# cure-lab/MagicDrive

Hardware: AMD Instinct MI355X
Metric: 6-view scenes/sec at 224x400, 50-step DDIM (higher is better)
Workload: dtype bf16; 1 GPU; configs[1]: 6-view 224x400, text-only conditioning (camera_param=None -> CFG off), 50-step DDIM, bf16; scenes_per_gpu=64, ddim_steps=50, scheduler=ddim, parallelism=scene-sharded x1, hipgraph=True, streams=2, output_type=latent

## Files before the change

### include/mdx.h

```cpp
#ifndef MDX_H_
#define MDX_H_

#include <stdint.h>

#ifdef __cplusplus
extern "C" {
#endif

#define MDX_OK 0
#define MDX_EINVAL (-1)
#define MDX_ELAUNCH (-2)
#define MDX_EUNSUPPORTED (-3)

#define MDX_ABI_VERSION 12

#define MDX_EPI_NONE 0
#define MDX_EPI_GEGLU 1
#define MDX_EPI_SILU 2

typedef struct MdxGemmDesc {
    const void* A; const void* W; void* C; const void* R;
    const float* bias; const float* temb; const int32_t* sel_ptr; float* ws;
    int64_t M, N, K;
    int64_t lda, ldw, ldc, ldr;
// ... 32 lines not shown
    const void* X; const void* Wt; void* Y; const void* R;
    const float* bias; const float* temb; const int32_t* sel_ptr; void* reserved_p;
    int64_t B, Hi, Wi, Cin, Ho, Wo, Cout;
    int64_t kh, kw, sh, sw, ph, pw;
    int64_t ldx, ldy, ldr;
    int64_t temb_sel_stride, temb_b_stride;
    int64_t epilogue, x_is_f32, y_is_f32, reserved0;
} MdxConvDirectDesc;
int mdx_conv2d_direct(const MdxConvDirectDesc* d, void* stream);

typedef struct MdxAttnDesc {
    const void* Q; const void* K; const void* Vt; void* O;
    const int32_t* kvmap; const int32_t* tk_dev;
    int64_t B, H, Tq, Tk, d, nsrc;
    int64_t ldq, sQ, ldk, sK, ldv, sV, ldo, sO;
    double scale;
    int64_t joint;
    int64_t q_prescaled;
    int64_t causal;
    int64_t v_rowmajor;
} MdxAttnDesc;
int mdx_attention_bf16(const MdxAttnDesc* d, void* stream);
int mdx_attention_ctx_rows_bf16(const MdxAttnDesc* d, void* stream);

typedef struct MdxGroupNormDesc {
    const void* X; void* Y; const float* gamma; const float* beta;
    int64_t B, HW, C, G, ldx, ldy;
    double eps;
    int64_t silu;
    float* ws; int64_t ws_bytes;
} MdxGroupNormDesc;
int mdx_groupnorm_bf16(const MdxGroupNormDesc* d, void* stream);

int mdx_groupnorm_resident_bf16(const MdxGroupNormDesc* d, void* stream);

typedef struct MdxLayerNormDesc {
    const void* X; void* Y; const float* gamma; const float* beta;
    int64_t M, C, ldx, ldy;
    double eps;
    int64_t reserved0;
} MdxLayerNormDesc;
int mdx_layernorm_bf16(const MdxLayerNormDesc* d, void* stream);

typedef struct MdxSoftmaxDesc {
    const float* X; void* Y;
    int64_t rows, T, ldx, ldy;
// ... 85 lines not shown
    int64_t n, group_elems, jump, n_rows, coef_ld, col_t, col_p, cfg, xin_c, xin_ld;
} MdxRenoiseDesc;
int mdx_latent_renoise_bf16(const MdxRenoiseDesc* d, void* stream);

#define MDX_OP_GEMM 1
#define MDX_OP_CONV 2
#define MDX_OP_CONV_DIRECT 3
#define MDX_OP_ATTN 4
#define MDX_OP_GROUPNORM 5
#define MDX_OP_LAYERNORM 6
#define MDX_OP_EW 7
#define MDX_OP_FOURIER 8
#define MDX_OP_GATHER 9
#define MDX_OP_TIMEEMB 10
#define MDX_OP_DDIM 11
#define MDX_OP_UNIPC 12
#define MDX_OP_SOFTMAX 13
#define MDX_OP_ATTN_ROWS 14
#define MDX_OP_GROUPNORM_RESIDENT 15
#define MDX_OP_GROUP_STATS 16
#define MDX_OP_SDPA 17
#define MDX_OP_LATENT_BLEND 18
#define MDX_OP_LATENT_RENOISE 19

#define MDX_DTYPE_BF16 0
#define MDX_DTYPE_F16 1

#define MDX_OP_BYTES 512
typedef struct MdxOp {
    int64_t opcode;
    int64_t dtype;
    unsigned char desc[MDX_OP_BYTES - 16];
} MdxOp;

int mdx_gemm_f16(const MdxGemmDesc* d, void* stream);
int mdx_conv2d_f16(const MdxConvDesc* d, void* stream);
int mdx_conv2d_direct_f16(const MdxConvDirectDesc* d, void* stream);
int mdx_attention_f16(const MdxAttnDesc* d, void* stream);
int mdx_groupnorm_f16(const MdxGroupNormDesc* d, void* stream);
int mdx_groupnorm_resident_f16(const MdxGroupNormDesc* d, void* stream);
int mdx_layernorm_f16(const MdxLayerNormDesc* d, void* stream);
int mdx_elementwise_f16(const MdxEwDesc* d, void* stream);
int mdx_fourier_embed_f16(const MdxFourierDesc* d, void* stream);
int mdx_gather_rows_f16(const MdxGatherDesc* d, void* stream);
int mdx_timestep_embedding_f16(const MdxTimeEmbDesc* d, void* stream);
int mdx_cfg_ddim_step_f16(const MdxDdimDesc* d, void* stream);
int mdx_cfg_unipc_step_f16(const MdxUniPCDesc* d, void* stream);
int mdx_softmax_rows_f16(const MdxSoftmaxDesc* d, void* stream);
int mdx_attention_ctx_rows_f16(const MdxAttnDesc* d, void* stream);
int mdx_group_stats_f16(const MdxStatsDesc* d, void* stream);
int mdx_sdpa_f16(const MdxSdpaDesc* d, void* stream);
int mdx_latent_blend_f16(const MdxBlendDesc* d, void* stream);
int mdx_latent_renoise_f16(const MdxRenoiseDesc* d, void* stream);

int mdx_program_run(const MdxOp* ops, int64_t n, void* stream);

int mdx_graph_create(const MdxOp* ops, int64_t n, void** graph_out);
int mdx_graph_launch(void* graph, void* stream);
int mdx_graph_destroy(void* graph);

int mdx_abi_version(void);
const char* mdx_build_id(void);
const char* mdx_last_error(void);
const char* mdx_last_kernel(void);
int mdx_set_option(const char* key, int64_t value);
int mdx_get_option(const char* key, int64_t* value_out);
const char* mdx_option_name(int64_t index);

int mdx_device_info(int64_t* out3);

#ifdef __cplusplus
}
#endif
#endif
```

### magicdrive_amd/_lib.py

```python
from __future__ import annotations

import ctypes as C
import os
from typing import Dict, List, Tuple

_HERE = os.path.dirname(os.path.abspath(__file__))
LIB_PATH = os.environ.get("MDX_LIB_PATH") or os.path.join(_HERE, "libmdx.so")

ABI_VERSION = 12

OP_GEMM, OP_CONV, OP_CONV_DIRECT, OP_ATTN, OP_GROUPNORM, OP_LAYERNORM = 1, 2, 3, 4, 5, 6
OP_EW, OP_FOURIER, OP_GATHER, OP_TIMEEMB, OP_DDIM, OP_UNIPC, OP_SOFTMAX = 7, 8, 9, 10, 11, 12, 13
OP_ATTN_ROWS = 14
OP_GROUPNORM_RESIDENT = 15
OP_GROUP_STATS = 16
OP_SDPA = 17
OP_LATENT_BLEND = 18
OP_LATENT_RENOISE = 19
OP_BYTES = 512

EPI_NONE, EPI_GEGLU, EPI_SILU = 0, 1, 2
EW_ADD, EW_COPY, EW_UPSAMPLE, EW_NCHW_TO_NHWC, EW_NHWC_TO_NCHW, EW_SILU, EW_SCALE = 1, 2, 3, 4, 5, 6, 7

P, I, D = C.c_void_p, C.c_int64, C.c_double


def _struct(name: str, fields: List[Tuple[str, object]]):
    return type(name, (C.Structure,), {"_fields_": fields})


def _f(kind, names: str):
    return [(n, kind) for n in names.split()]


MdxGemmDesc = _struct("MdxGemmDesc", _f(P, "A W C R bias temb sel_ptr ws") + _f(I, "M N K lda ldw ldc ldr batch sA sW sC sR "
                      "temb_sel_stride temb_b_stride rows_per_b epilogue splitk c_is_f32 ws_bytes") + _f(P, "Vt") + _f(I, "vt_from vt_T vt_ld vt_stride")
                      + _f(D, "ln_eps") + _f(P, "ln_csum ln_scratch") + _f(P, "rowstat_out") + _f(I, "rowstat_parts") + _f(P, "ln_stats") + _f(I, "ln_stats_parts") + _f(P, "Wq"))
MdxConvDesc = _struct("MdxConvDesc", _f(P, "X Wt Y R bias temb sel_ptr ws") + _f(I, "B Hi Wi Cin Ho Wo Cout kh kw sh sw ph pw "
                      "ldx ldy ldr temb_sel_stride temb_b_stride epilogue splitk ws_bytes upsample2x"))
MdxConvDirectDesc = _struct("MdxConvDirectDesc", _f(P, "X Wt Y R bias temb sel_ptr reserved_p") + _f(I, "B Hi Wi Cin Ho Wo Cout kh kw sh sw ph pw "
                            "ldx ldy ldr temb_sel_stride temb_b_stride epilogue x_is_f32 y_is_f32 reserved0"))
# ... 12 lines not shown

MdxSoftmaxDesc = _struct("MdxSoftmaxDesc", _f(P, "X Y") + _f(I, "rows T ldx ldy") + _f(D, "scale") + _f(I, "reserved0"))
MdxStatsDesc = _struct("MdxStatsDesc", _f(P, "X out row_dev") + _f(I, "G n sG n_rows f32"))
MdxSdpaDesc = _struct("MdxSdpaDesc", _f(P, "Q K V O klen_dev") + _f(I, "B H Tq Tk d ldq sQ ldk sK ldv sV ldo sO") + _f(D, "scale") + _f(I, "causal"))
MdxBlendDesc = _struct("MdxBlendDesc", _f(P, "x cond noise mask coef step_ptr x_in") + _f(I, "n mask_elems coef_ld col_a col_s last_step cfg xin_c xin_ld"))
MdxRenoiseDesc = _struct("MdxRenoiseDesc", _f(P, "x x_in coef step_ptr visit_ptr seeds") + _f(I, "n group_elems jump n_rows coef_ld col_t col_p cfg xin_c xin_ld"))
DESC_OF_OP = {
    OP_GEMM: MdxGemmDesc, OP_CONV: MdxConvDesc, OP_CONV_DIRECT: MdxConvDirectDesc, OP_ATTN: MdxAttnDesc,
    OP_GROUPNORM: MdxGroupNormDesc, OP_LAYERNORM: MdxLayerNormDesc, OP_EW: MdxEwDesc, OP_FOURIER: MdxFourierDesc,
    OP_GATHER: MdxGatherDesc, OP_TIMEEMB: MdxTimeEmbDesc, OP_DDIM: MdxDdimDesc, OP_UNIPC: MdxUniPCDesc, OP_SOFTMAX: MdxSoftmaxDesc,
}
DTYPE_BF16, DTYPE_F16 = 0, 1
ENTRY_OF_OP = {
    OP_GEMM: "mdx_gemm_bf16", OP_CONV: "mdx_conv2d_bf16", OP_CONV_DIRECT: "mdx_conv2d_direct", OP_ATTN: "mdx_attention_bf16",
    OP_GROUPNORM: "mdx_groupnorm_bf16", OP_LAYERNORM: "mdx_layernorm_bf16", OP_EW: "mdx_elementwise",
    OP_FOURIER: "mdx_fourier_embed", OP_GATHER: "mdx_gather_rows", OP_TIMEEMB: "mdx_timestep_embedding", OP_DDIM: "mdx_cfg_ddim_step",
    OP_UNIPC: "mdx_cfg_unipc_step", OP_SOFTMAX: "mdx_softmax_rows",
    OP_ATTN_ROWS: "mdx_attention_ctx_rows_bf16",
    OP_GROUPNORM_RESIDENT: "mdx_groupnorm_resident_bf16",
    OP_GROUP_STATS: "mdx_group_stats_bf16",
    OP_SDPA: "mdx_sdpa_bf16",
    OP_LATENT_BLEND: "mdx_latent_blend_bf16",
    OP_LATENT_RENOISE: "mdx_latent_renoise_bf16",
}
def entry_name(opcode: int, dtype: int = DTYPE_BF16) -> str:
    n = ENTRY_OF_OP[opcode]
    if dtype == DTYPE_BF16:
        return n
    return (n[:-5] if n.endswith("_bf16") else n) + "_f16"


EXPORTS = sorted(set(ENTRY_OF_OP.values()) | {entry_name(o, DTYPE_F16) for o in ENTRY_OF_OP} | {
    "mdx_program_run", "mdx_graph_create", "mdx_graph_launch", "mdx_graph_destroy",
    "mdx_abi_version", "mdx_build_id", "mdx_last_error", "mdx_last_kernel", "mdx_device_info", "mdx_set_option", "mdx_get_option", "mdx_option_name"})


class MdxOp(C.Structure):
    _fields_ = [("opcode", I), ("dtype", I), ("desc", C.c_ubyte * (OP_BYTES - 16))]


assert C.sizeof(MdxOp) == OP_BYTES
for _d in list(DESC_OF_OP.values()) + [MdxStatsDesc, MdxSdpaDesc, MdxBlendDesc, MdxRenoiseDesc]:
    assert C.sizeof(_d) <= OP_BYTES - 16 and C.sizeof(_d) % 8 == 0


class MdxError(RuntimeError):
# ... 142 lines not shown
```

### magicdrive_amd/csrc/api.hip

```cpp
#include <cstring>
#include <mutex>
#include <set>
#include <utility>
#include "launch.h"
#include "options.h"
#include <atomic>
#include <cstdlib>

namespace mdx_rt {
char* error_buffer() {
    static thread_local char buf[512] = {0};
    return buf;
}
char* kernel_tag_buffer() {
    static thread_local char buf[128] = {0};
    return buf;
}
int ensure_dyn_smem(const void* kernel, size_t bytes, const char* what) {
    static std::mutex mu;
    static std::set<std::pair<const void*, int>> done;
    int dev = 0;
    hipError_t e = hipGetDevice(&dev);
    if (e != hipSuccess) return mdx::set_error(MDX_ELAUNCH, "hipGetDevice: %s", hipGetErrorString(e));
    std::lock_guard<std::mutex> lk(mu);
// ... 58 lines not shown
static int run_op(const MdxOp* op, hipStream_t st) {
    const void* d = op->desc;
    if (op->dtype == MDX_DTYPE_F16) {
        switch (op->opcode) {
            case MDX_OP_GEMM: return mdx_gemm_f16((const MdxGemmDesc*)d, st);
            case MDX_OP_CONV: return mdx_conv2d_f16((const MdxConvDesc*)d, st);
            case MDX_OP_CONV_DIRECT: return mdx_conv2d_direct_f16((const MdxConvDirectDesc*)d, st);
            case MDX_OP_ATTN: return mdx_attention_f16((const MdxAttnDesc*)d, st);
            case MDX_OP_GROUPNORM: return mdx_groupnorm_f16((const MdxGroupNormDesc*)d, st);
            case MDX_OP_GROUPNORM_RESIDENT: return mdx_groupnorm_resident_f16((const MdxGroupNormDesc*)d, st);
            case MDX_OP_LAYERNORM: return mdx_layernorm_f16((const MdxLayerNormDesc*)d, st);
            case MDX_OP_EW: return mdx_elementwise_f16((const MdxEwDesc*)d, st);
            case MDX_OP_FOURIER: return mdx_fourier_embed_f16((const MdxFourierDesc*)d, st);
            case MDX_OP_GATHER: return mdx_gather_rows_f16((const MdxGatherDesc*)d, st);
            case MDX_OP_TIMEEMB: return mdx_timestep_embedding_f16((const MdxTimeEmbDesc*)d, st);
            case MDX_OP_DDIM: return mdx_cfg_ddim_step_f16((const MdxDdimDesc*)d, st);
            case MDX_OP_UNIPC: return mdx_cfg_unipc_step_f16((const MdxUniPCDesc*)d, st);
            case MDX_OP_SOFTMAX: return mdx_softmax_rows_f16((const MdxSoftmaxDesc*)d, st);
            case MDX_OP_ATTN_ROWS: return mdx_attention_ctx_rows_f16((const MdxAttnDesc*)d, st);
            case MDX_OP_GROUP_STATS: return mdx_group_stats_f16((const MdxStatsDesc*)d, st);
            case MDX_OP_SDPA: return mdx_sdpa_f16((const MdxSdpaDesc*)d, st);
            case MDX_OP_LATENT_BLEND: return mdx_latent_blend_f16((const MdxBlendDesc*)d, st);
            case MDX_OP_LATENT_RENOISE: return mdx_latent_renoise_f16((const MdxRenoiseDesc*)d, st);
            default: return set_error(MDX_EINVAL, "unknown opcode %ld", (long)op->opcode);
        }
    }
    if (op->dtype != MDX_DTYPE_BF16) return set_error(MDX_EINVAL, "MdxOp.dtype %ld: 0 (bf16) or 1 (fp16)", (long)op->dtype);
    switch (op->opcode) {
        case MDX_OP_GEMM: return mdx_gemm_bf16((const MdxGemmDesc*)d, st);
        case MDX_OP_CONV: return mdx_conv2d_bf16((const MdxConvDesc*)d, st);
        case MDX_OP_CONV_DIRECT: return mdx_conv2d_direct((const MdxConvDirectDesc*)d, st);
        case MDX_OP_ATTN: return mdx_attention_bf16((const MdxAttnDesc*)d, st);
        case MDX_OP_GROUPNORM: return mdx_groupnorm_bf16((const MdxGroupNormDesc*)d, st);
        case MDX_OP_GROUPNORM_RESIDENT: return mdx_groupnorm_resident_bf16((const MdxGroupNormDesc*)d, st);
        case MDX_OP_LAYERNORM: return mdx_layernorm_bf16((const MdxLayerNormDesc*)d, st);
        case MDX_OP_EW: return mdx_elementwise((const MdxEwDesc*)d, st);
        case MDX_OP_FOURIER: return mdx_fourier_embed((const MdxFourierDesc*)d, st);
        case MDX_OP_GATHER: return mdx_gather_rows((const MdxGatherDesc*)d, st);
        case MDX_OP_TIMEEMB: return mdx_timestep_embedding((const MdxTimeEmbDesc*)d, st);
        case MDX_OP_DDIM: return mdx_cfg_ddim_step((const MdxDdimDesc*)d, st);
        case MDX_OP_UNIPC: return mdx_cfg_unipc_step((const MdxUniPCDesc*)d, st);
        case MDX_OP_SOFTMAX: return mdx_softmax_rows((const MdxSoftmaxDesc*)d, st);
        case MDX_OP_ATTN_ROWS: return mdx_attention_ctx_rows_bf16((const MdxAttnDesc*)d, st);
        case MDX_OP_GROUP_STATS: return mdx_group_stats_bf16((const MdxStatsDesc*)d, st);
        case MDX_OP_SDPA: return mdx_sdpa_bf16((const MdxSdpaDesc*)d, st);
        case MDX_OP_LATENT_BLEND: return mdx_latent_blend_bf16((const MdxBlendDesc*)d, st);
        case MDX_OP_LATENT_RENOISE: return mdx_latent_renoise_bf16((const MdxRenoiseDesc*)d, st);
        default: return set_error(MDX_EINVAL, "unknown opcode %ld", (long)op->opcode);
    }
}

extern "C" int mdx_program_run(const MdxOp* ops, int64_t n, void* stream) {
    if (!ops && n > 0) return set_error(MDX_EINVAL, "mdx_program_run: null program");
    for (int64_t i = 0; i < n; ++i) {
        int rc = run_op(&ops[i], (hipStream_t)stream);
        if (rc != MDX_OK) {
            char tmp[400];
            strncpy(tmp, error_buffer(), sizeof(tmp) - 1);
            tmp[sizeof(tmp) - 1] = 0;
            return set_error(rc, "op %ld (opcode %ld): %s", (long)i, (long)ops[i].opcode, tmp);
        }
    }
    return MDX_OK;
}

struct GraphHandle {
    hipGraph_t graph;
    hipGraphExec_t exec;
};

// ... 61 lines not shown
```

### magicdrive_amd/csrc/options.h

```cpp
#pragma once
#include <cstdint>

namespace mdx_rt {
int64_t opt(int id);
}

namespace mdx {

#define MDX_OPTIONS(X) \
    X(ATTN_SWZ, 2, "XCD-aware block order of attention.hip: 0 off, 1 per (view, head), 2 per view (all heads of a view on one XCD)") \
    X(ATTN_NW4_BLOCKS, 256L, "attention.hip: 4-wave workgroups from this many blocks") \
    X(ATTN_NW8_BLOCKS, (1L << 40), "attention.hip: 8-wave workgroups from this many blocks") \
    X(ATTN_NW, 0, "force the waves per workgroup of attention.hip (0 = heuristic)") \
    X(ATTN2, 1, "attention2.hip for head dim 40") \
    X(ATTN3, 0, "only in `make ATTN3=1` builds: tools/attn3/attention3.hip (permute-free P, QK of the next kv tile beside this tile's softmax) for the head-dim-40 FOLD launches: self, cross-view, joint") \
    X(ATTN3_WGS, 0, "attention3.hip: persistent workgroups per XCD (0 = automatic: two per CU)") \
    X(ATTN2_PF, 1, "attention2.hip, head dim 40 FOLD 32-query form: permute-free P (PV on 32x32x16 MFMAs, K rows permuted so that a lane's scores are its PV operand)") \
    X(ATTN2_D80, 2, "attention2.hip for head dim 80: 0 never, 1 always, 2 only the two-source cross-view form") \
    X(ATTN2_FOLD, 1, "attention2.hip: subtract the running maximum inside the QK MFMA when Q is pre-scaled (head dim 40)") \
    X(ATTN2_RES, 1, "attention2.hip: kv sequences of <= 3 tiles (text context) resident in LDS, one workgroup per (view, head) walks the query blocks: 0 off, 1 for launches of >= 1024 (view, head) pairs, 2 whenever supported") \
    X(ATTN2_VIEWMAP, 1, "attention2.hip block order: 1 = all heads and query blocks of a view on one XCD (a row's 128-byte lines are shared by the heads), 0 = per (view, head)") \
    X(ATTN2_QT, 0, "32-query tiles per wave in attention2.hip: 0 = automatic (2; 1 for one-source FOLD launches), 1 / 2 = force") \
    X(CONV_OUT_WS, 1, "direct conv with Cout <= 4 and a long K (conv_out): weight-stationary K-parallel kernel (weights in registers, 16 pixels per wave)") \
    X(GEMM_SWZ, 1, "XCD-aware tile order of the generic kernel") \
// ... 10 lines not shown
    X(XL_GEGLU320, 0, "K = 320 GEGLU on the 256-wide XL tile instead of gemm_ws.hip") \
    X(GEMM_BM256, 0, "generic 256x128 8-wave tile from M >= value (0 = never)") \
    X(GEMM_TIMING, 0, "s_memtime stamps of the generic kernel into the op workspace") \
    X(GEMM_BK, 64, "generic tile slab depth (64 or 32)") \
    X(GEMM_FLATTEN, 1, "batched shared-A GEMM as ONE col_split XL launch") \
    X(CONV_CIMAJOR, 1, "channel-block-major K order of implicit-GEMM convs") \
    X(WS_SLOTS, 512, "workgroup slots the gemm_ws M walkers are sized for") \
    X(XL_TIMING, 0, "per-workgroup s_memtime stamps into the op workspace") \
    X(GN_REVERSE, 1, "two-stage GroupNorm: statistics pass reads the tensor back to front (Infinity-Cache reuse between producer / passes)") \
    X(GN_FINALIZE_CHUNKS, 16, "two-stage GroupNorm: with more chunks per image than this the chunk partials are combined once by gn_finalize_kernel (0 = always in the apply pass)") \
    X(GN_ONE_KERNEL_ELEMS, (4L << 20), "GroupNorm tensors of at most this many elements (all images) take the one-launch kernel (one workgroup per (image, group)) instead of the two streaming passes") \
    X(GN_TWO_STAGE, 1, "streaming two-stage GroupNorm for maps >= 32768 elements") \
    X(GN_RESIDENT, 1, "register-resident one-read GroupNorm (gn_resident_kernel, an op of its own: MDX_OP_GROUPNORM_RESIDENT): 0 off (the engine emits none, the entry point refuses), 1 where gn_route.h says so (tensors above GN_ONE_KERNEL_ELEMS), 2 whenever the kernel can serve the shape") \
    X(GN_RESIDENT_K, 0, "force the groups per workgroup of gn_resident_kernel (0 = gn_route.h: the widest block that fits; tools/gn_bench.py sweeps it)") \
    X(XL_PERSIST, 1, "256x256 XL GEMMs (plain / GEGLU, optional residual) on the persistent kernel gemm_xlp_kernel") \
    X(XD, 0, "W-direct persistent GEMM (gemm_xd.hip: weights global -> registers, finished tile stored under the next tile's main loop) for the 256x256 XL GEMMs whose descriptor carries Wq (K % 128 == 0, K >= 640); bit-identical to gemm_xlp_kernel, measured 0.89-1.04x of it (profiles/r06_xd_ab.log): off by default") \
    X(XL_RASTER, 2, "XL tile order: 0 row-major, 1 XCD-strided M-tiles, 2 XCD-blocked (M-group x N-group panels per XCD)") \
    X(XL_GM, 0, "XL_RASTER 2: force the M-tiles per panel (0 = cost model, xl_layout.h: raster_shape)") \
    X(XL_GN, 0, "XL_RASTER 2: force the N-tiles per panel (0 = cost model)") \
    X(STREAMS, 2, "host side (pipeline): HIP streams a pipe() call spreads its scene chunks over (chunks of >= 16 scenes, one plan + hipGraph each)") \
    X(PLAN_CACHE, 6, "host side (pipeline): sampler plans (captured graphs + buffers) kept per pipeline (LRU); a multi-stream call pins one plan per chunk") \
    X(CHECK_TIMESTEPS, 0, "host side (schedulers): 1 = a device-resident timestep that is not in the scheduler's list raises (one sync per step) instead of poisoning the sample with NaN") \
    X(LN_FUSE, 1, "MdxGemmDesc.ln_eps: 1 = gemm_ws.hip normalises the rows in-kernel, 0 = always normalise into ln_scratch first (A/B)") \
    X(LN_STATS, 1, "MdxGemmDesc.rowstat_out / ln_stats: 1 = row statistics travel from the producer's store phase to the fused LayerNorm, 0 = round-5 behaviour (nothing emitted, in-kernel sums, GEGLU through ln_scratch) (A/B)")

enum Opt : int {
#define MDX_OPT_ENUM(key, dflt, doc) OPT_##key,
    MDX_OPTIONS(MDX_OPT_ENUM)
#undef MDX_OPT_ENUM
    OPT_COUNT
};

using mdx_rt::opt;

}
```

### magicdrive_amd/engine.py

```python
from __future__ import annotations

from typing import Dict, List, Optional, Sequence, Tuple

import torch

from . import _lib as L
from . import gn_route as GR
from . import ops as O
from . import packing as PK
from .networks.spec import heads_at

BF16, F32 = torch.bfloat16, torch.float32


def q_prescale(head_dim: int) -> float:
    return float(head_dim) ** -0.5 * 1.4426950408889634


class PackedNet:

    def __init__(self, sd: Dict[str, torch.Tensor], device, dtype=BF16):
        assert dtype in (torch.bfloat16, torch.float16), "the kernels take bf16 or fp16 operands (fp32 accumulate)"
        self.sd = sd
        self.device = device
        self.dtype = dtype
        self.cache: Dict[Tuple, torch.Tensor] = {}

    def has(self, key: str) -> bool:
        return key in self.sd

# ... 192 lines not shown
    def bhwc(self):
        return self.parent.bhwc[..., self.c0:self.c0 + self.C]

    @property
    def btc(self):
        return self.parent.btc[..., self.c0:self.c0 + self.C]


def upsample_conv_folds(device, fold, Hi: int, Wi: int, Ho: int, Wo: int, cin: int, B: int = 0, ldx: int = 0) -> bool:
    if fold is None:
        fold = torch.device(device).type == "cuda"
    if not (bool(fold) and cin % 64 == 0 and Hi * Wi + 256 < (1 << 24) and PK.upsample_fold_ok(Hi, Ho) and PK.upsample_fold_ok(Wi, Wo)):
        return False
    if B and (Ho != 2 * Hi or Wo != 2 * Wi) and (B * Hi * Wi + Wi + 2) * (ldx or cin) * 2 >= 0x7fff0000:
        return False
    return True


class Builder:

    fold_upsample = None

    gn_resident = None

    def __init__(self, cfg, device, n_views: int, n_cam: int, ws_mb: int = 64, dtype=BF16):
        self.cfg = cfg
        self.device = device
        self.B = n_views
        self.n_cam = n_cam
        self.dtype = dtype
        self.pool = Pool(device, dtype)
        self.ops: List[object] = []
        self.ctx_tk_dev: Optional[torch.Tensor] = None
        self.ctx_tk_per_view = False
        self.ws = torch.empty(ws_mb * 1024 * 1024 // 4, dtype=F32, device=device)
        self.groups = cfg["norm_num_groups"]
        self.eps = cfg["norm_eps"]
        pair = cfg["neighboring_view_pair"]
        pair = {int(k): [int(x) for x in v] for k, v in pair.items()}
        self.nattn = cfg.get("neighboring_attn_type", "add")
        if self.nattn not in ("add", "concat", "self"):
            raise NotImplementedError(f"Unknown type: {self.nattn}")
        counts = [len(pair[c]) for c in range(n_cam)]
        self.xv_counts: Optional[List[int]] = None
        self.xv_bo_scale = 1.0
        if self.nattn == "add":
# ... 144 lines not shown
        M = B * T
        if fuse_ln:
            n1 = self.pool.get(tuple(h.shape))
            ao = self.self_like_attention(net, pre + "attn1.", h, B, T, C, heads, False, name + ".attn1", ln_pre=pre + "norm1.", ln_scratch=n1, ln_stats=h_stats)
            self.pool.put(h_stats)
        else:
            n1 = self.layernorm(net, pre + "norm1.", h, name + ".norm1")
            ao = self.self_like_attention(net, pre + "attn1.", n1, B, T, C, heads, False, name + ".attn1")
        self.pool.put(n1)
        s1 = self.rowstat(M) if fuse_ln else None
        h1 = self.gemm(ao, net.lin(pre + "attn1.to_out.0.weight"), C, bias=net.vec(pre + "attn1.to_out.0.bias"), R=h, rowstat=s1, name=name + ".attn1.out")
        self.pool.put(ao); self.pool.put(h)
        if fuse_ln:
            n2 = self.pool.get(tuple(h1.shape))
            w, b, cs = net.ln_lin([pre + "attn2.to_q.weight"], pre + "norm2.", (q_prescale(C // heads),))
            q2 = self.gemm(h1, w, C, bias=b, ln_eps=1e-5, ln_csum=cs, ln_scratch=n2, ln_stats=s1, name=name + ".attn2.ln+q")
            self.pool.put(s1)
        else:
            n2 = self.layernorm(net, pre + "norm2.", h1, name + ".norm2")
            q2 = self.gemm(n2, net.lin(pre + "attn2.to_q.weight", q_prescale(C // heads)), C, name=name + ".attn2.q")
        self.pool.put(n2)
        Kc, Vtc, S = ctx_kv[pre + "attn2."]
        ao2 = self.pool.get((B * T, C))
        self.emit(O.Attn(q2.view(B, T, C), Kc, Vtc, ao2.view(B, T, C), heads=heads, Tk=S, scale=(C // heads) ** -0.5, q_prescaled=True,
                         tk_dev=None if self.ctx_tk_per_view else self.ctx_tk_dev, tk_rows=self.ctx_tk_dev if self.ctx_tk_per_view else None,
                         name=name + ".attn2"))
        self.pool.put(q2)
        has4 = net.has(pre + "attn4.to_q.weight")
        fold3 = fuse_ln and self.FOLD_NORM3 and not (has4 and self.xv_counts is not None)
        s2 = self.rowstat(M) if (fuse_ln and (has4 or fold3)) else None
        h2 = self.gemm(ao2, net.lin(pre + "attn2.to_out.0.weight"), C, bias=net.vec(pre + "attn2.to_out.0.bias"), R=h1, rowstat=s2, name=name + ".attn2.out")
        self.pool.put(ao2); self.pool.put(h1)
        s3 = s2
        if has4:
            if fuse_ln:
                n4 = self.pool.get(tuple(h2.shape))
                ao4 = self.self_like_attention(net, pre + "attn4.", h2, B, T, C, heads, True, name + ".attn4", ln_pre=pre + "norm4.", ln_scratch=n4, ln_stats=s2)
                self.pool.put(s2)
            else:
                n4 = self.layernorm(net, pre + "norm4.", h2, name + ".norm4")
                ao4 = self.self_like_attention(net, pre + "attn4.", n4, B, T, C, heads, True, name + ".attn4")
            self.pool.put(n4)
            bo_scale = self.xv_bo_scale
            zero_linear = net.has(pre + "connector.weight")
            alpha_key = pre + "connector.alpha" if net.has(pre + "connector.alpha") else None
            if self.xv_counts is not None:
                if zero_linear:
                    wf, tab = net.folded_affine_rows(pre + "connector.weight", pre + "connector.bias", pre + "attn4.to_out.0.weight", pre + "attn4.to_out.0.bias", self.xv_counts)
                else:
# ... 208 lines not shown
```

### magicdrive_amd/ops.py

```python
from __future__ import annotations

from dataclasses import dataclass, field
from typing import Optional

import torch

from . import _lib as L

BF16 = torch.bfloat16
F16 = torch.float16
H16 = (BF16, F16)
F32 = torch.float32


def _p(t: Optional[torch.Tensor]):
    return None if t is None else t.data_ptr()


def _chk(cond: bool, msg: str):
    if not cond:
        raise ValueError(msg)


def _rows2d(t: torch.Tensor):
# ... 234 lines not shown
            if self.ws is not None:
                d.ws = _p(self.ws); d.ws_bytes = self.ws.numel() * self.ws.element_size()
        return self.opcode, d


@dataclass
class Attn:
    Q: torch.Tensor
    K: torch.Tensor
    Vt: torch.Tensor
    O: torch.Tensor
    heads: int
    Tk: int
    scale: float
    kvmap: Optional[torch.Tensor] = None
    nsrc: int = 1
    name: str = ""
    joint: bool = False
    q_prescaled: bool = False
    causal: bool = False
    v_rowmajor: bool = False
    tk_dev: Optional[torch.Tensor] = None
    tk_rows: Optional[torch.Tensor] = None
    opcode = L.OP_ATTN

    def lower(self):
        Q, K, Vt, O = self.Q, self.K, self.Vt, self.O
        B, Tq, Cc = Q.shape
        _chk(Q.stride(2) == 1 and K.stride(2) == 1 and O.stride(2) == 1 and Vt.stride(2) == 1, f"attn {self.name}: inner strides")
        if self.v_rowmajor:
            _chk(Cc % self.heads == 0 and K.shape[2] == Cc and Vt.shape[2] == Cc and O.shape == Q.shape, f"attn {self.name}: shapes")
            _chk(K.shape[1] == self.Tk and Vt.shape[1] == self.Tk and Vt.shape[0] == K.shape[0], f"attn {self.name}: kv shapes")
        else:
            _chk(not self.causal, f"attn {self.name}: causal needs v_rowmajor")
            _chk(Cc % self.heads == 0 and K.shape[2] == Cc and Vt.shape[1] == Cc and O.shape == Q.shape, f"attn {self.name}: shapes")
            _chk(K.shape[1] == self.Tk and Vt.shape[2] >= self.Tk and Vt.shape[0] == K.shape[0], f"attn {self.name}: kv shapes")
        d = L.MdxAttnDesc()
        d.Q, d.K, d.Vt, d.O = _p(Q), _p(K), _p(Vt), _p(O)
        if self.kvmap is not None:
            _chk(self.kvmap.dtype == torch.int32 and self.kvmap.numel() == B * self.nsrc, f"attn {self.name}: kvmap")
            d.kvmap = _p(self.kvmap)
        else:
            _chk(self.nsrc == 1 and K.shape[0] == B, f"attn {self.name}: identity kv map needs Bkv == B")
        d.B, d.H, d.Tq, d.Tk, d.d, d.nsrc = B, self.heads, Tq, self.Tk, Cc // self.heads, self.nsrc
        d.ldq, d.sQ = Q.stride(1), Q.stride(0)
        d.ldk, d.sK = K.stride(1), K.stride(0)
        d.ldv, d.sV = Vt.stride(1), Vt.stride(0)
        d.ldo, d.sO = O.stride(1), O.stride(0)
        d.scale = float(self.scale)
        d.joint = int(self.joint)
        d.q_prescaled = int(self.q_prescaled)
        d.causal, d.v_rowmajor = int(self.causal), int(self.v_rowmajor)
        if self.tk_dev is not None:
            _chk(self.tk_dev.dtype == torch.int32 and self.tk_dev.numel() == 1 and self.tk_dev.device == Q.device,
                 f"attn {self.name}: tk_dev must be one int32 on the device of Q")
            _chk(self.nsrc == 1 and self.kvmap is None and not self.joint and not self.causal and not self.v_rowmajor,
                 f"attn {self.name}: tk_dev serves one source, no joint softmax, no causal mask, the V^T operand")
            d.tk_dev = _p(self.tk_dev)
        opcode = self.opcode
        if self.tk_rows is not None:
            _chk(self.tk_dev is None, f"attn {self.name}: tk_rows and tk_dev are mutually exclusive")
            _chk(self.tk_rows.dtype == torch.int32 and self.tk_rows.dim() == 1 and self.tk_rows.numel() == B and self.tk_rows.is_contiguous()
                 and self.tk_rows.device == Q.device, f"attn {self.name}: tk_rows must be int32 [B={B}], contiguous, on the device of Q")
            _chk(self.nsrc == 1 and self.kvmap is None and not self.joint and not self.causal and not self.v_rowmajor,
                 f"attn {self.name}: tk_rows serves one source, no joint softmax, no causal mask, the V^T operand")
            d.tk_dev = _p(self.tk_rows)
            opcode = L.OP_ATTN_ROWS
        _chk(self.nsrc >= 1 and (self.nsrc <= 8 if self.joint else self.nsrc <= 2), f"attn {self.name}: nsrc={self.nsrc} (joint={self.joint})")
        return opcode, d


@dataclass
class GroupNorm:
    X: torch.Tensor
    Y: torch.Tensor
    gamma: torch.Tensor
    beta: torch.Tensor
    groups: int
    eps: float
    silu: bool = False
    ws: Optional[torch.Tensor] = None
    name: str = ""
    opcode = L.OP_GROUPNORM

    def lower(self):
        B, HW, Cc = self.X.shape
        _chk(self.X.stride(2) == 1 and self.Y.stride(2) == 1 and self.Y.shape == self.X.shape, f"gn {self.name}: layout")
        _chk(B == 1 or (self.X.stride(0) == HW * self.X.stride(1) and self.Y.stride(0) == HW * self.Y.stride(1)), f"gn {self.name}: batch stride")
        _chk(self.gamma.dtype == F32 and self.beta.dtype == F32 and self.gamma.numel() == Cc, f"gn {self.name}: affine")
        d = L.MdxGroupNormDesc()
        d.X, d.Y, d.gamma, d.beta = _p(self.X), _p(self.Y), _p(self.gamma), _p(self.beta)
# ... 447 lines not shown
```

Measured before the change: 7.774 scenes/s.

## Add dedicated whole-row text cross-attention kernel for short key lengths

```diff
diff --git a/include/mdx.h b/include/mdx.h
--- a/include/mdx.h
+++ b/include/mdx.h
@@ -78,6 +78,7 @@
 } MdxAttnDesc;
 int mdx_attention_bf16(const MdxAttnDesc* d, void* stream);
 int mdx_attention_ctx_rows_bf16(const MdxAttnDesc* d, void* stream);
+int mdx_attention_text_bf16(const MdxAttnDesc* d, void* stream);
 
 typedef struct MdxGroupNormDesc {
     const void* X; void* Y; const float* gamma; const float* beta;
@@ -209,6 +210,7 @@
 #define MDX_OP_SDPA 17
 #define MDX_OP_LATENT_BLEND 18
 #define MDX_OP_LATENT_RENOISE 19
+#define MDX_OP_ATTN_TEXT 20
 
 #define MDX_DTYPE_BF16 0
 #define MDX_DTYPE_F16 1
@@ -239,6 +241,7 @@
 int mdx_sdpa_f16(const MdxSdpaDesc* d, void* stream);
 int mdx_latent_blend_f16(const MdxBlendDesc* d, void* stream);
 int mdx_latent_renoise_f16(const MdxRenoiseDesc* d, void* stream);
+int mdx_attention_text_f16(const MdxAttnDesc* d, void* stream);
 
 int mdx_program_run(const MdxOp* ops, int64_t n, void* stream);
 
diff --git a/magicdrive_amd/_lib.py b/magicdrive_amd/_lib.py
--- a/magicdrive_amd/_lib.py
+++ b/magicdrive_amd/_lib.py
@@ -17,6 +17,7 @@
 OP_SDPA = 17
 OP_LATENT_BLEND = 18
 OP_LATENT_RENOISE = 19
+OP_ATTN_TEXT = 20
 OP_BYTES = 512
 
 EPI_NONE, EPI_GEGLU, EPI_SILU = 0, 1, 2
@@ -75,6 +76,7 @@
     OP_SDPA: "mdx_sdpa_bf16",
     OP_LATENT_BLEND: "mdx_latent_blend_bf16",
     OP_LATENT_RENOISE: "mdx_latent_renoise_bf16",
+    OP_ATTN_TEXT: "mdx_attention_text_bf16",
 }
 def entry_name(opcode: int, dtype: int = DTYPE_BF16) -> str:
     n = ENTRY_OF_OP[opcode]
diff --git a/magicdrive_amd/attn_text_route.py b/magicdrive_amd/attn_text_route.py
--- /dev/null
+++ b/magicdrive_amd/attn_text_route.py
@@ -0,0 +1,36 @@
+from __future__ import annotations
+
+ATT_GROUP_CH = 320
+ATT_MAX_TK = 96
+ATT_MIN_TQ = 256
+ATT_MIN_BH = 1024
+
+
+def attn_text_supported(B: int, H: int, Tq: int, Tk: int, d: int, nsrc: int, has_kvmap: bool, joint: bool, causal: bool, v_rowmajor: bool,
+                        has_tk_dev: bool, q_prescaled: bool, ldq: int, sQ: int, ldk: int, sK: int, ldv: int, sV: int, ldo: int, sO: int,
+                        alignment: int, mode: int = 1) -> bool:
+    if mode <= 0:
+        return False
+    if nsrc != 1 or has_kvmap or joint or causal:
+        return False
+    if v_rowmajor or has_tk_dev or not q_prescaled:
+        return False
+    if not (H == 8 and d in (40, 80)):
+        return False
+    if B < 1 or Tq < 1 or Tk < 1 or Tk > ATT_MAX_TK:
+        return False
+    C = H * d
+    if ldq < C or ldo < C or ldk < C or ldv < Tk:
+        return False
+    if any(v % 8 for v in (ldq, sQ, ldo, sO, ldk, sK, ldv, sV)):
+        return False
+    if alignment < 16:
+        return False
+    tiles = (Tq + 31) // 32
+    if B > 0x7fffffff // (tiles * 2):
+        return False
+    if Tq * max(ldq, ldo) >= (1 << 30):
+        return False
+    if mode >= 2:
+        return True
+    return Tq >= ATT_MIN_TQ and B * H >= ATT_MIN_BH
diff --git a/magicdrive_amd/csrc/api.hip b/magicdrive_amd/csrc/api.hip
--- a/magicdrive_amd/csrc/api.hip
+++ b/magicdrive_amd/csrc/api.hip
@@ -104,6 +104,7 @@
             case MDX_OP_SDPA: return mdx_sdpa_f16((const MdxSdpaDesc*)d, st);
             case MDX_OP_LATENT_BLEND: return mdx_latent_blend_f16((const MdxBlendDesc*)d, st);
             case MDX_OP_LATENT_RENOISE: return mdx_latent_renoise_f16((const MdxRenoiseDesc*)d, st);
+            case MDX_OP_ATTN_TEXT: return mdx_attention_text_f16((const MdxAttnDesc*)d, st);
             default: return set_error(MDX_EINVAL, "unknown opcode %ld", (long)op->opcode);
         }
     }
@@ -128,6 +129,7 @@
         case MDX_OP_SDPA: return mdx_sdpa_bf16((const MdxSdpaDesc*)d, st);
         case MDX_OP_LATENT_BLEND: return mdx_latent_blend_bf16((const MdxBlendDesc*)d, st);
         case MDX_OP_LATENT_RENOISE: return mdx_latent_renoise_bf16((const MdxRenoiseDesc*)d, st);
+        case MDX_OP_ATTN_TEXT: return mdx_attention_text_bf16((const MdxAttnDesc*)d, st);
         default: return set_error(MDX_EINVAL, "unknown opcode %ld", (long)op->opcode);
     }
 }
diff --git a/magicdrive_amd/csrc/attention_text.hip b/magicdrive_amd/csrc/attention_text.hip
--- /dev/null
+++ b/magicdrive_amd/csrc/attention_text.hip
@@ -0,0 +1,276 @@
+#include "common.h"
+#include "launch.h"
+#include "options.h"
+#include "attn_text_route.h"
+
+#if defined(MDX_F16) && MDX_F16
+#define mdx_attention_text_bf16 mdx_attention_text_f16
+#endif
+
+namespace mdx {
+
+struct AttnTextParams {
+    const bf16_t* Q; const bf16_t* K; const bf16_t* Vt; bf16_t* O;
+    int Tq, Tk, tkp, ntile;
+    long ldq, sQ, ldk, sK, ldv, sV, ldo, sO;
+    long total;
+};
+
+constexpr int AT_NW = 8, AT_NT = AT_NW * 64;
+constexpr int AT_CH = mdx_route::ATT_GROUP_CH;
+constexpr int AT_KSTR = AT_CH + 8;
+constexpr int AT_OSTR = 80;
+constexpr int AT_OTILE = 32 * AT_OSTR;
+__host__ __device__ constexpr int at_vstr(int tkp) { return tkp + 8; }
+__host__ __device__ constexpr int at_lds_bytes(int tkp) { return tkp * AT_KSTR * 2 + AT_CH * at_vstr(tkp) * 2 + AT_NW * AT_OTILE; }
+
+#define RLIVE(sub) (((sub) == NSUB - 1 && (NK16 & 1)) ? 8 : 16)
+template <int D, int NK16, bool FULL>
+__global__ __launch_bounds__(AT_NT) void attn_text_kernel(AttnTextParams p) {
+    static_assert(D == 40 || D == 80, "head dim");
+    constexpr int HG = AT_CH / D;
+    constexpr int NG = 8 / HG;
+    constexpr int D16 = (D + 15) / 16;
+    constexpr int DT = (D + 31) / 32;
+    constexpr bool RAGGED = (D % 16) != 0;
+    extern __shared__ __attribute__((aligned(16))) unsigned char at_smem[];
+
+    const int tid = threadIdx.x, lane = tid & 63;
+    const int wave = __builtin_amdgcn_readfirstlane(tid >> 6);
+    const int half = lane >> 5, col = lane & 31;
+    constexpr int NSUB = (NK16 + 1) / 2;
+    constexpr int tkp = NSUB * 32, vstr = at_vstr(tkp), nsub = NSUB;
+    bf16_t* Ks = (bf16_t*)at_smem;
+    bf16_t* Vs = (bf16_t*)(at_smem + tkp * AT_KSTR * 2);
+    unsigned char* Os = at_smem + tkp * AT_KSTR * 2 + AT_CH * vstr * 2 + wave * AT_OTILE;
+
+    const long T0 = (long)blockIdx.x * p.total / gridDim.x, T1 = (long)(blockIdx.x + 1) * p.total / gridDim.x;
+
+    Frag8 qf[HG][D16];
+    auto load_q = [&](int hh, const unsigned char* qb, unsigned off, unsigned off_rag) {
+#pragma unroll
+        for (int ks = 0; ks < D16; ++ks) {
+            if (RAGGED && ks == D16 - 1) qf[hh][ks].u = *(const uint4*)(qb + off_rag + hh * D * 2);
+            else qf[hh][ks].u = *(const uint4*)(qb + off + hh * D * 2 + ks * 32);
+        }
+    };
+    unsigned o_off[3]; int o_row[3];
+#pragma unroll
+    for (int j = 0; j < 3; ++j) {
+        const int idx = lane + 64 * j, row = idx / 5;
+        o_row[j] = idx < 160 ? row : 0x7fffffff; o_off[j] = (unsigned)(row * (int)p.ldo * 2 + (idx - row * 5) * 16);
+    }
+
+    for (long seg = T0 / p.ntile; seg * p.ntile < T1; ++seg) {
+        const long b = seg / NG;
+        const int ch0 = (int)(seg - b * NG) * AT_CH;
+        const long s0 = seg * p.ntile;
+        const int hi = (int)((T1 < s0 + p.ntile ? T1 : s0 + p.ntile) - s0);
+        int t = (int)((T0 > s0 ? T0 : s0) - s0) + wave;
+        const unsigned char* qbase = (const unsigned char*)(p.Q + b * p.sQ + ch0);
+        unsigned char* obase = (unsigned char*)(p.O + b * p.sO + ch0);
+        auto tile_row0 = [&](int tile) { return FULL ? min(tile * 32, p.Tq - 32) : tile * 32; };
+        auto q_off = [&](int tile) { const int q = tile_row0(tile) + col; return (unsigned)((q < p.Tq ? q : p.Tq - 1) * (int)p.ldq * 2); };
+        if (t < hi) {
+            const unsigned qo = q_off(t);
+#pragma unroll
+            for (int hh = 0; hh < HG; ++hh) load_q(hh, qbase, qo + half * 16, qo + (half ? 0 : (D16 - 1) * 32));
+        }
+        __syncthreads();
+        {
+            const bf16_t* kbase = p.K + b * p.sK + ch0;
+            constexpr int KC = AT_KSTR / 8;
+            for (int c = tid; c < tkp * KC; c += AT_NT) {
+                const int row = c / KC, cc = c - row * KC;
+                uint4 v = make_uint4(0, 0, 0, 0);
+                if (row < p.Tk && cc < AT_CH / 8) v = *(const uint4*)(kbase + (long)row * p.ldk + cc * 8);
+                *(uint4*)(Ks + row * AT_KSTR + cc * 8) = v;
+            }
+            const bf16_t* vbase = p.Vt + b * p.sV + (long)ch0 * p.ldv;
+            const int nch = tkp >> 3;
+            for (int c = tid; c < AT_CH * nch; c += AT_NT) {
+                const int row = c / nch, kv0 = (c - row * nch) * 8;
+                Frag8 v;
+                v.u = make_uint4(0, 0, 0, 0);
+                if (kv0 < p.Tk) {
+                    v.u = *(const uint4*)(vbase + (long)row * p.ldv + kv0);
+                    if (kv0 + 8 > p.Tk) {
+#pragma unroll
+                        for (int e = 0; e < 8; ++e)
+                            if (kv0 + e >= p.Tk) v.h[e] = 0;
+                    }
+                }
+                bf16_t* dst = Vs + row * vstr + (kv0 & ~15) + ((kv0 & 8) >> 1);
+                *(uint2*)dst = v.d2[0];
+                *(uint2*)(dst + 8) = v.d2[1];
+            }
+        }
+        __syncthreads();
+
+        for (; t < hi; t += AT_NW) {
+            const bool has_next = t + AT_NW < hi;
+            const unsigned qn = has_next ? q_off(t + AT_NW) : 0u;
+            const unsigned qn0 = has_next ? qn + half * 16 : 0u, qn1 = has_next ? qn + (half ? 0 : (D16 - 1) * 32) : 0u;
+            unsigned char* otile = obase + (long)tile_row0(t) * p.ldo * 2;
+            const int qleft = p.Tq - t * 32;
+#pragma unroll
+            for (int hh = 0; hh < HG; ++hh) {
+                __builtin_amdgcn_sched_barrier(0);
+                f32x16_t sacc[NSUB];
+#pragma unroll
+                for (int sub = 0; sub < NSUB; ++sub) {
+                    if (sub < nsub) {
+                        if (sub) __builtin_amdgcn_sched_barrier(0);
+#pragma unroll
+                        for (int r = 0; r < 16; ++r) sacc[sub][r] = 0.f;
+                        const bf16_t* kr = Ks + (sub * 32 + col) * AT_KSTR + hh * D + half * 8;
+#pragma unroll
+                        for (int ks = 0; ks < D16; ++ks) {
+                            Frag8 kf, qv = qf[hh][ks];
+                            kf.u = *(const uint4*)(kr + ks * 16);
+                            if (RAGGED && ks == D16 - 1 && half) qv.u = make_uint4(0, 0, 0, 0);
+                            sacc[sub] = MDX_MFMA_32x32x16(kf.v, qv.v, sacc[sub]);
+                        }
+                    }
+                }
+                load_q(hh, qbase, qn0, qn1);
+                float mx = -INFINITY;
+#pragma unroll
+                for (int sub = 0; sub < NSUB; ++sub) {
+                    if (sub < nsub) {
+                        if (sub == nsub - 1 && p.Tk < tkp) {
+#pragma unroll
+                            for (int r = 0; r < RLIVE(sub); ++r)
+                                if (sub * 32 + mfma32_row(r, lane) >= p.Tk) sacc[sub][r] = -INFINITY;
+                        }
+#pragma unroll
+                        for (int r = 0; r < RLIVE(sub); ++r) mx = fmaxf(mx, sacc[sub][r]);
+                    }
+                }
+                mx = fmaxf(mx, __shfl_xor(mx, 32, 64));
+                f32x2_t psum2 = {0.f, 0.f};
+                const f32x2_t mx2 = {mx, mx};
+                unsigned pk[NSUB][8];
+#pragma unroll
+                for (int sub = 0; sub < NSUB; ++sub) {
+                    if (sub < nsub) {
+#pragma unroll
+                        for (int r = 0; r < RLIVE(sub); r += 2) {
+                            const f32x2_t dv = f32x2_t{sacc[sub][r], sacc[sub][r + 1]} - mx2;
+                            const f32x2_t pv = {__builtin_amdgcn_exp2f(dv.x), __builtin_amdgcn_exp2f(dv.y)};
+                            psum2 += pv;
+                            pk[sub][r >> 1] = pack2bf(pv.x, pv.y);
+                        }
+                    }
+                }
+                const float psum = psum2.x + psum2.y;
+                const float inv = 1.0f / (psum + __shfl_xor(psum, 32, 64));
+                const f32x2_t inv2 = {inv, inv};
+                f32x16_t oacc[DT];
+#pragma unroll
+                for (int i = 0; i < DT; ++i)
+#pragma unroll
+                    for (int r = 0; r < 16; ++r) oacc[i][r] = 0.f;
+                const bf16_t* vlane = Vs + col * vstr + 8 * half;
+#pragma unroll
+                for (int kstep = 0; kstep < NK16; ++kstep) {
+                    __builtin_amdgcn_sched_barrier(0);
+                    const int sub = kstep >> 1, kk = kstep & 1;
+                    if (sub < nsub) {
+                        Frag8 pf;
+                        pf.u = make_uint4(pk[sub][kk * 4], pk[sub][kk * 4 + 1], pk[sub][kk * 4 + 2], pk[sub][kk * 4 + 3]);
+#pragma unroll
+                        for (int i = 0; i < DT; ++i) {
+                            const bf16_t* vr = vlane + (hh * D + i * 32) * vstr + kstep * 16;
+                            Frag8 vf;
+                            vf.u = *(const uint4*)(vr);
+                            oacc[i] = MDX_MFMA_32x32x16(vf.v, pf.v, oacc[i]);
+                        }
+                    }
+                }
+#pragma unroll
+                for (int rd = 0; rd < D / 40; ++rd) {
+                    __builtin_amdgcn_wave_barrier();
+#pragma unroll
+                    for (int i = 0; i < DT; ++i)
+#pragma unroll
+                        for (int g = 0; g < 4; ++g) {
+                            const int base = i * 32 + 8 * g;
+                            if (base < rd * 40 || base >= rd * 40 + 40) continue;
+                            uint2 ov;
+                            const f32x2_t lo = f32x2_t{oacc[i][4 * g], oacc[i][4 * g + 1]} * inv2, hi2 = f32x2_t{oacc[i][4 * g + 2], oacc[i][4 * g + 3]} * inv2;
+                            ov.x = pack2bf(lo.x, lo.y);
+                            ov.y = pack2bf(hi2.x, hi2.y);
+                            *(uint2*)(Os + col * AT_OSTR + (base - rd * 40 + 4 * half) * 2) = ov;
+                        }
+                    __builtin_amdgcn_wave_barrier();
+#pragma unroll
+                    for (int j = 0; j < 3; ++j) {
+                        const uint4 ov = *(const uint4*)(Os + ((lane + 64 * j) & 255) * 16);
+                        if (FULL ? (j < 2 || lane < 32) : o_row[j] < qleft) *(uint4*)(otile + o_off[j] + (hh * D + rd * 40) * 2) = ov;
+                    }
+                }
+            }
+        }
+    }
+}
+
+#undef RLIVE
+template <int D, int NK16>
+static int launch_attn_text_n(const AttnTextParams& p, int grid, const char* tag, hipStream_t st) {
+    constexpr int lds = at_lds_bytes((NK16 + 1) / 2 * 32);
+    if (p.Tq >= 32) {
+        MDX_NEED(ensure_dyn_smem((const void*)attn_text_kernel<D, NK16, true>, lds, tag));
+        hipLaunchKernelGGL((attn_text_kernel<D, NK16, true>), dim3((unsigned)grid), dim3(AT_NT), lds, st, p);
+    } else {
+        MDX_NEED(ensure_dyn_smem((const void*)attn_text_kernel<D, NK16, false>, lds, tag));
+        hipLaunchKernelGGL((attn_text_kernel<D, NK16, false>), dim3((unsigned)grid), dim3(AT_NT), lds, st, p);
+    }
+    return check_launch(tag);
+}
+template <int D>
+static int launch_attn_text(const AttnTextParams& p, int grid, const char* tag, hipStream_t st) {
+    switch ((p.Tk + 15) / 16) {
+        case 1: return launch_attn_text_n<D, 1>(p, grid, tag, st);
+        case 2: return launch_attn_text_n<D, 2>(p, grid, tag, st);
+        case 3: return launch_attn_text_n<D, 3>(p, grid, tag, st);
+        case 4: return launch_attn_text_n<D, 4>(p, grid, tag, st);
+        case 5: return launch_attn_text_n<D, 5>(p, grid, tag, st);
+        default: return launch_attn_text_n<D, 6>(p, grid, tag, st);
+    }
+}
+
+static int attn_text(const MdxAttnDesc* a, hipStream_t st, const char* op) {
+    if (!a) return set_error(MDX_EINVAL, "%s: null descriptor", op);
+    if (!a->Q || !a->K || !a->Vt || !a->O) return set_error(MDX_EINVAL, "%s: null operand", op);
+    const uintptr_t bits = (uintptr_t)a->Q | (uintptr_t)a->K | (uintptr_t)a->Vt | (uintptr_t)a->O;
+    const mdx_route::AttnTextIn in = {a->B, a->H, a->Tq, a->Tk, a->d, a->nsrc, a->kvmap != nullptr, a->joint != 0, a->causal != 0, a->v_rowmajor != 0,
+                                      a->tk_dev != nullptr, a->q_prescaled == 1, a->ldq, a->sQ, a->ldk, a->sK, a->ldv, a->sV, a->ldo, a->sO,
+                                      (bits & 15) ? 1 : 16};
+    const mdx_route::AttnTextOpts o = {(int)opt(OPT_ATTN_TEXT)};
+    if (!mdx_route::attn_text_supported(in, o))
+        return set_error(MDX_EINVAL, "%s: not a descriptor this kernel takes (csrc/attn_text_route.h; option ATTN_TEXT=%d): B=%ld H=%ld Tq=%ld Tk=%ld d=%ld nsrc=%ld "
+                         "kvmap=%d tk_dev=%d joint=%ld causal=%ld v_rowmajor=%ld q_prescaled=%ld ldq=%ld ldk=%ld ldv=%ld ldo=%ld", op, o.ATTN_TEXT, (long)a->B, (long)a->H,
+                         (long)a->Tq, (long)a->Tk, (long)a->d, (long)a->nsrc, a->kvmap != nullptr, a->tk_dev != nullptr, (long)a->joint, (long)a->causal, (long)a->v_rowmajor,
+                         (long)a->q_prescaled, (long)a->ldq, (long)a->ldk, (long)a->ldv, (long)a->ldo);
+    AttnTextParams p;
+    p.Q = (const bf16_t*)a->Q; p.K = (const bf16_t*)a->K; p.Vt = (const bf16_t*)a->Vt; p.O = (bf16_t*)a->O;
+    p.Tq = (int)a->Tq; p.Tk = (int)a->Tk; p.tkp = (int)((a->Tk + 31) / 32) * 32; p.ntile = (int)((a->Tq + 31) / 32);
+    p.ldq = a->ldq; p.sQ = a->sQ; p.ldk = a->ldk; p.sK = a->sK; p.ldv = a->ldv; p.sV = a->sV; p.ldo = a->ldo; p.sO = a->sO;
+    p.total = a->B * (a->H * a->d / AT_CH) * (long)p.ntile;
+    int dev = 0, ncu = 0;
+    hipError_t e = hipGetDevice(&dev);
+    if (e == hipSuccess) e = hipDeviceGetAttribute(&ncu, hipDeviceAttributeMultiprocessorCount, dev);
+    if (e != hipSuccess || ncu <= 0) return set_error(MDX_ELAUNCH, "%s: compute-unit count: %s", op, hipGetErrorString(e));
+    const long want = (p.total + AT_NW - 1) / AT_NW;
+    const int grid = (int)(want < ncu ? want : ncu);
+    return a->d == 40 ? launch_attn_text<40>(p, grid, "attn_text_kernel<40>", st) : launch_attn_text<80>(p, grid, "attn_text_kernel<80>", st);
+}
+
+}
+
+using namespace mdx;
+
+extern "C" int mdx_attention_text_bf16(const MdxAttnDesc* a, void* stream) {
+    return attn_text(a, (hipStream_t)stream, MDX_F16 ? "mdx_attention_text_f16" : "mdx_attention_text_bf16");
+}
diff --git a/magicdrive_amd/csrc/attn_text_route.h b/magicdrive_amd/csrc/attn_text_route.h
--- /dev/null
+++ b/magicdrive_amd/csrc/attn_text_route.h
@@ -0,0 +1,35 @@
+#pragma once
+
+namespace mdx_route {
+
+constexpr int ATT_GROUP_CH = 320;
+constexpr int ATT_MAX_TK = 96;
+constexpr long ATT_MIN_TQ = 256;
+constexpr long ATT_MIN_BH = 1024;
+
+struct AttnTextIn {
+    long B, H, Tq, Tk, d, nsrc;
+    bool has_kvmap, joint, causal, v_rowmajor, has_tk_dev, q_prescaled;
+    long ldq, sQ, ldk, sK, ldv, sV, ldo, sO;
+    long alignment;
+};
+struct AttnTextOpts { int ATTN_TEXT; };
+
+inline bool attn_text_supported(const AttnTextIn& p, const AttnTextOpts& o) {
+    if (o.ATTN_TEXT <= 0) return false;
+    if (p.nsrc != 1 || p.has_kvmap || p.joint || p.causal) return false;
+    if (p.v_rowmajor || p.has_tk_dev || !p.q_prescaled) return false;
+    if (!(p.H == 8 && (p.d == 40 || p.d == 80))) return false;
+    if (p.B < 1 || p.Tq < 1 || p.Tk < 1 || p.Tk > ATT_MAX_TK) return false;
+    const long C = p.H * p.d;
+    if (p.ldq < C || p.ldo < C || p.ldk < C || p.ldv < p.Tk) return false;
+    if ((p.ldq % 8) || (p.sQ % 8) || (p.ldo % 8) || (p.sO % 8) || (p.ldk % 8) || (p.sK % 8) || (p.ldv % 8) || (p.sV % 8)) return false;
+    if (p.alignment < 16) return false;
+    const long tiles = (p.Tq + 31) / 32;
+    if (p.B > 0x7fffffffL / (tiles * 2)) return false;
+    if (p.Tq * (p.ldq > p.ldo ? p.ldq : p.ldo) >= (1L << 30)) return false;
+    if (o.ATTN_TEXT >= 2) return true;
+    return p.Tq >= ATT_MIN_TQ && p.B * p.H >= ATT_MIN_BH;
+}
+
+}
diff --git a/magicdrive_amd/csrc/options.h b/magicdrive_amd/csrc/options.h
--- a/magicdrive_amd/csrc/options.h
+++ b/magicdrive_amd/csrc/options.h
@@ -56,7 +56,8 @@
     X(PLAN_CACHE, 6, "host side (pipeline): sampler plans (captured graphs + buffers) kept per pipeline (LRU); a multi-stream call pins one plan per chunk") \
     X(CHECK_TIMESTEPS, 0, "host side (schedulers): 1 = a device-resident timestep that is not in the scheduler's list raises (one sync per step) instead of poisoning the sample with NaN") \
     X(LN_FUSE, 1, "MdxGemmDesc.ln_eps: 1 = gemm_ws.hip normalises the rows in-kernel, 0 = always normalise into ln_scratch first (A/B)") \
-    X(LN_STATS, 1, "MdxGemmDesc.rowstat_out / ln_stats: 1 = row statistics travel from the producer's store phase to the fused LayerNorm, 0 = round-5 behaviour (nothing emitted, in-kernel sums, GEGLU through ln_scratch) (A/B)")
+    X(LN_STATS, 1, "MdxGemmDesc.rowstat_out / ln_stats: 1 = row statistics travel from the producer's store phase to the fused LayerNorm, 0 = round-5 behaviour (nothing emitted, in-kernel sums, GEGLU through ln_scratch) (A/B)") \
+    X(ATTN_TEXT, 1, "whole-row text cross-attention (attn_text_kernel, an op of its own: MDX_OP_ATTN_TEXT): 0 off (the engine emits none, the entry point refuses), 1 where attn_text_route.h says so (Tq >= 256 and B * H >= 1024), 2 whenever the kernel can serve the descriptor")
 
 enum Opt : int {
 #define MDX_OPT_ENUM(key, dflt, doc) OPT_##key,
diff --git a/magicdrive_amd/engine.py b/magicdrive_amd/engine.py
--- a/magicdrive_amd/engine.py
+++ b/magicdrive_amd/engine.py
@@ -6,6 +6,7 @@
 
 from . import _lib as L
 from . import gn_route as GR
+from . import attn_text_route as ATR
 from . import ops as O
 from . import packing as PK
 from .networks.spec import heads_at
@@ -244,6 +245,8 @@
     fold_upsample = None
 
     gn_resident = None
+
+    attn_text = None
 
     def __init__(self, cfg, device, n_views: int, n_cam: int, ws_mb: int = 64, dtype=BF16):
         self.cfg = cfg
@@ -434,9 +437,17 @@
         self.pool.put(n2)
         Kc, Vtc, S = ctx_kv[pre + "attn2."]
         ao2 = self.pool.get((B * T, C))
-        self.emit(O.Attn(q2.view(B, T, C), Kc, Vtc, ao2.view(B, T, C), heads=heads, Tk=S, scale=(C // heads) ** -0.5, q_prescaled=True,
+        mode = self.attn_text
+        if mode is None:
+            mode = L.get_option("ATTN_TEXT") if torch.device(self.device).type == "cuda" else 0
+        q3, o3 = q2.view(B, T, C), ao2.view(B, T, C)
+        text = mode > 0 and self.ctx_tk_dev is None and ATR.attn_text_supported(
+            B=B, H=heads, Tq=T, Tk=S, d=C // heads, nsrc=1, has_kvmap=False, joint=False, causal=False, v_rowmajor=False, has_tk_dev=False, q_prescaled=True,
+            ldq=q3.stride(1), sQ=q3.stride(0), ldk=Kc.stride(1), sK=Kc.stride(0), ldv=Vtc.stride(1), sV=Vtc.stride(0), ldo=o3.stride(1), sO=o3.stride(0),
+            alignment=16 if (q3.data_ptr() | Kc.data_ptr() | Vtc.data_ptr() | o3.data_ptr()) % 16 == 0 else 1, mode=mode)
+        self.emit(O.Attn(q3, Kc, Vtc, o3, heads=heads, Tk=S, scale=(C // heads) ** -0.5, q_prescaled=True,
                          tk_dev=None if self.ctx_tk_per_view else self.ctx_tk_dev, tk_rows=self.ctx_tk_dev if self.ctx_tk_per_view else None,
-                         name=name + ".attn2"))
+                         text=text, name=name + ".attn2"))
         self.pool.put(q2)
         has4 = net.has(pre + "attn4.to_q.weight")
         fold3 = fuse_ln and self.FOLD_NORM3 and not (has4 and self.xv_counts is not None)
diff --git a/magicdrive_amd/ops.py b/magicdrive_amd/ops.py
--- a/magicdrive_amd/ops.py
+++ b/magicdrive_amd/ops.py
@@ -280,6 +280,7 @@
     v_rowmajor: bool = False
     tk_dev: Optional[torch.Tensor] = None
     tk_rows: Optional[torch.Tensor] = None
+    text: bool = False
     opcode = L.OP_ATTN
 
     def lower(self):
@@ -325,6 +326,9 @@
             d.tk_dev = _p(self.tk_rows)
             opcode = L.OP_ATTN_ROWS
         _chk(self.nsrc >= 1 and (self.nsrc <= 8 if self.joint else self.nsrc <= 2), f"attn {self.name}: nsrc={self.nsrc} (joint={self.joint})")
+        if self.text:
+            _chk(self.tk_dev is None and self.tk_rows is None, f"attn {self.name}: the whole-row text kernel takes a host-side key count")
+            opcode = L.OP_ATTN_TEXT
         return opcode, d
 
 
```

Result: no change. 7.789 scenes/s (median of 6 runs) (+0.2%).
